# sidfeels/cosmos-predict2.5

Measured on AMD Instinct MI355X. Metric: frames/sec, Predict2.5-2B Image2World 720p×121f, 35 UniPC steps, CP=1/8, higher is better.
Workload: dtype bf16

## Files before the change

cosmos-predict2.5_amd/csrc/attn_wide.hip:

```cpp
#include "attn_common.h"

namespace cp25attn {
namespace {

constexpr int kAheadWq = 2;
constexpr int kRingWq = kAheadWq + 1;
static_assert(kWqThreads == 4 * 64, "one wave per SIMD");

constexpr int wq_stage(int nq) { return 17 * nq; }
constexpr int wq_frag(int nq, int m) { return m < nq ? -1 : (m - nq) / nq; }
constexpr int wq_qb(int nq, int m) { return m < nq ? m : (m - nq) % nq; }
constexpr bool wq_read_gap(int nq, int m) { return m >= nq && (m - nq) % nq == 0; }
constexpr int wq_sm_op(int nq, int m) {
  if (wq_read_gap(nq, m)) return -1;
  int idx = 0;
  for (int x = 0; x < m; ++x) idx += !wq_read_gap(nq, x);
  return idx < 12 * nq ? idx : -1;
}
constexpr int wq_sm_count(int nq) {
  int n = 0;
  for (int m = 0; m < wq_stage(nq); ++m) n += wq_sm_op(nq, m) >= 0;
  return n;
}
static_assert(wq_sm_count(5) == 60 && wq_sm_count(6) == 72, "every softmax instruction has a gap");
#ifdef CP25_WQ_PARENT_LOOP
#define CP25_WQ_ITER_TILES 1
#undef CP25_WQ_NO_PAD_FETCH
#undef CP25_WQ_GAP_RSRC
#endif
#ifndef CP25_WQ_ITER_TILES
#define CP25_WQ_ITER_TILES 2
#endif
constexpr int wq_iter_tiles(int) { return CP25_WQ_ITER_TILES; }
#ifdef CP25_WQ_NO_PAD_FETCH
constexpr bool kWqPadFetch = false;
#else
constexpr bool kWqPadFetch = true;
#endif
#ifdef CP25_WQ_GAP_RSRC
constexpr bool kWqHeadRsrc = false;
#else
constexpr bool kWqHeadRsrc = true;
#endif
constexpr int kWqImg = kKBuf16;
static_assert(kKBuf16 == kVBuf16, "K and V images of one size");
constexpr int wq_dma_n(int it) { return it == 1 ? 10 : 18; }
constexpr int wq_dma_at(int nq, int it, int M) {
  const int st = M / wq_stage(nq), m = M % wq_stage(nq);
  if (st >= 2 * it || !wq_read_gap(nq, m)) return -1;
  const int F = 16 * st + wq_frag(nq, m);
  return F < wq_dma_n(it) ? F : -1;
}
constexpr int wq_m0_at(int nq, int it, int M) { return wq_dma_at(nq, it, M + 1); }
constexpr int kWqNoFetch = 0x7ffffff0;

__device__ __forceinline__ u32x4 tile_rsrc(const char* base, int64_t sl, int rows) {
  const uint64_t p = (uint64_t)base;
  const unsigned n = rows > 0 ? (unsigned)((rows - 1) * sl * 2 + 2 * kD) : 0u;
  return u32x4{(unsigned)p, (unsigned)(p >> 32) & 0xffffu, n, 0x00020000u};
}

#define WQ_MFMA "v_mfma_f32_16x16x32_bf16 "

template <int kNQ, int kMode, int kTail = 0>
__global__ void __launch_bounds__(kWqThreads, 1) attn_fwd_wq(AttnArgs a) {
  static_assert(kMode == 0 || kMode == 1, "kMode: 0 fixed shift, 1 zero shift");
  static_assert(kNQ >= 4 && kNQ <= 6, "query blocks per wave");
  constexpr int kIT = wq_iter_tiles(kNQ);
  static_assert(kIT == 1 || kIT == 2, "tiles per iteration");
  constexpr int kBuf = kIT * kWqImg;
  constexpr int VB0 = 2 * kBuf;
  static_assert(4 * kBuf <= 163840, "the CU's LDS");
  __shared__ __attribute__((aligned(16))) char smem[4 * kBuf];
  constexpr bool kInit = kMode != 1;
  constexpr int kPar = kIT == 1 ? 1 : 0;
  constexpr int kND = wq_dma_n(kIT);
  constexpr int kR = kRingWq;
  constexpr int kRowsW = 16 * kNQ;
  constexpr int kRowsG = 4 * kRowsW;
  constexpr int kNS = wq_stage(kNQ);
  constexpr int kQA = (256 - 36 * kNQ - 4) / 16 < kNQ ? (256 - 36 * kNQ - 4) / 16 : kNQ;

  const int tile = xcd_remap(blockIdx.x, gridDim.x);
  const int qblk = tile % a.nqb;
  const int bhs = tile / a.nqb;
  const int split = bhs % a.nsplit, bh = bhs / a.nsplit;
  const int b = bh / a.H, h = bh % a.H;
  const int key0 = split * a.tps * kKBlk;
  const int Lk = min(a.Lk - key0, a.tps * kKBlk);
  const int ntk = (Lk + kKBlk - 1) / kKBlk;
  const int tid = threadIdx.x;
  const int lane = tid & 63;
  const int wave = __builtin_amdgcn_readfirstlane(tid >> 6);
  const int c16 = lane & 15;
  const int g = lane >> 4;
  const int row_w = qblk * kRowsG + wave * kRowsW;

  const unsigned short* qp = a.q + b * a.q_sb + h * a.q_sh;
  const char* const kbase = (const char*)(a.k + b * a.k_sb + h * a.k_sh + (int64_t)key0 * a.k_sl);
  const char* const vbase = (const char*)(a.v + b * a.v_sb + h * a.v_sh + (int64_t)key0 * a.v_sl);

  const int wave5 = kIT == 1 ? wave : (wave & 1);
  const int img5 = kIT == 1 ? 0 : (wave >> 1);
  int dk[5], dv[5];
#pragma unroll
  for (int j = 0; j < 5; ++j) {
    const int bb = 1024 * ((j < 4 ? wave : wave5) + 4 * j) + 16 * lane;
    const int row = bb / kKStride16, cb = bb - row * kKStride16;
    dk[j] = cb < 2 * kD ? row * (int)(a.k_sl * 2) + cb : (kWqPadFetch ? 0 : kWqNoFetch);
    dv[j] = cb < 2 * kD ? row * (int)(a.v_sl * 2) + cb : (kWqPadFetch ? 0 : kWqNoFetch);
  }
  const unsigned lds_wave = (unsigned)(uintptr_t)(lds_char_ptr)smem + 1024u * (unsigned)wave;
  const unsigned lds_wave5 =
      (unsigned)(uintptr_t)(lds_char_ptr)smem + 1024u * (unsigned)wave5 + (unsigned)kWqImg * (unsigned)img5;
  auto k_rsrc = [&](int t) __attribute__((always_inline)) {
    return tile_rsrc(kbase + (int64_t)t * kKBlk * a.k_sl * 2, a.k_sl, min(Lk - t * kKBlk, kKBlk));
  };
  auto v_rsrc = [&](int t) __attribute__((always_inline)) {
    return tile_rsrc(vbase + (int64_t)t * kKBlk * a.v_sl * 2, a.v_sl, min(Lk - t * kKBlk, kKBlk));
  };
  auto set_m0 = [&](unsigned dst, auto OFFC) __attribute__((always_inline)) {
    asm volatile("s_add_u32 m0, %0, %1" ::"s"(dst), "i"(decltype(OFFC)::value) : "memory", "scc");
  };
  auto dma_load = [&](const u32x4& rs, int off) __attribute__((always_inline)) {
    asm volatile("buffer_load_dwordx4 %0, %1, 0 offen lds" ::"v"(off), "s"(rs) : "memory");
  };
  auto dma_piece = [&](const u32x4& rs, int off, unsigned dst, auto OFFC) __attribute__((always_inline)) {
    set_m0(dst, OFFC);
    asm volatile("s_nop 4" ::: "memory");
    dma_load(rs, off);
  };
  auto dma_img = [&](const u32x4& rs, const int* offs, unsigned at) __attribute__((always_inline)) {
    static_for<4>([&](auto JC) __attribute__((always_inline)) {
      dma_piece(rs, offs[decltype(JC)::value], lds_wave + at, std::integral_constant<int, 4096 * decltype(JC)::value>{});
    });
  };
  auto dma_buf = [&](auto rsrc, const int* offs, int t0, unsigned at) __attribute__((always_inline)) {
    if constexpr (kIT == 1) {
      const u32x4 rs = rsrc(t0);
      dma_img(rs, offs, at);
      if (wave < 2) dma_piece(rs, offs[4], lds_wave + at, std::integral_constant<int, 16384>{});
    } else {
      const u32x4 rs0 = rsrc(t0), rs1 = rsrc(t0 + 1);
      dma_img(rs0, offs, at);
      dma_img(rs1, offs, at + (unsigned)kWqImg);
      if (wave < 2) dma_piece(rs0, offs[4], lds_wave5 + at, std::integral_constant<int, 16384>{});
      else dma_piece(rs1, offs[4], lds_wave5 + at, std::integral_constant<int, 16384>{});
    }
  };

  constexpr unsigned kK0At = (unsigned)(((kPar + 1) & 1) * kBuf + (kIT - 1) * kWqImg);
  {
    const u32x4 rs = k_rsrc(0);
    dma_img(rs, dk, kK0At);
    if (wave < 2) dma_piece(rs, dk[4], lds_wave + kK0At, std::integral_constant<int, 16384>{});
  }
  dma_buf(k_rsrc, dk, 1, (unsigned)((kPar & 1) * kBuf));
  dma_buf(v_rsrc, dv, 0, (unsigned)VB0);

  bf16x8 qa[kNQ][4];
#pragma unroll
  for (int qb = 0; qb < kNQ; ++qb) {
    const int r = row_w + 16 * qb + c16;
    const unsigned short* src = qp + (int64_t)min(r, a.Lq - 1) * a.q_sl + 8 * g;
#pragma unroll
    for (int s = 0; s < 4; ++s) qa[qb][s] = *reinterpret_cast<const bf16x8*>(src + 32 * s);
  }
  if (a.qn_w != nullptr) {
    bf16x8 wv[4];
#pragma unroll
    for (int s = 0; s < 4; ++s) wv[s] = *reinterpret_cast<const bf16x8*>(a.qn_w + 32 * s + 8 * g);
    const bool rope = a.qn_cos != nullptr;
    const f32x2 scale2 = {a.qn_scale, a.qn_scale};
#pragma unroll
    for (int qb = 0; qb < kNQ; ++qb) {
      const int r = row_w + 16 * qb + c16;
      f32x4 rc[2][2], rsn[2][2];
      if (rope) {
        const int64_t t0 = (a.qn_row0 + min(r, a.Lq - 1)) * 64 + 8 * g;
#pragma unroll
        for (int s1 = 0; s1 < 2; ++s1)
#pragma unroll
          for (int hf = 0; hf < 2; ++hf) {
            rc[s1][hf] = *reinterpret_cast<const f32x4*>(a.qn_cos + t0 + 32 * s1 + 4 * hf);
            rsn[s1][hf] = *reinterpret_cast<const f32x4*>(a.qn_sin + t0 + 32 * s1 + 4 * hf);
          }
      }
      f32x2 x[4][4];
#pragma unroll
      for (int s = 0; s < 4; ++s)
#pragma unroll
        for (int q = 0; q < 4; ++q)
          x[s][q] = f32x2{static_cast<float>(qa[qb][s][2 * q]), static_cast<float>(qa[qb][s][2 * q + 1])};
      f32x2 c01[8], c23[8];
#pragma unroll
      for (int e = 0; e < 8; ++e) {
        c01[e] = f32x2{x[0][e >> 1][e & 1], x[1][e >> 1][e & 1]};
        c23[e] = f32x2{x[2][e >> 1][e & 1], x[3][e >> 1][e & 1]};
      }
      const f32x2 p01 = hn2_sumsq8(c01), p23 = hn2_sumsq8(c23);
      const f32x2 aa = p01 + p23;
      float ss = aa.x + aa.y;
      ss += __shfl_xor(ss, 32);
      ss += __shfl_xor(ss, 16);
      const float rstd = hn_rstd(ss, a.qn_eps);
      const f32x2 rstd2 = {rstd, rstd};
#pragma unroll
      for (int s = 0; s < 4; ++s)
#pragma unroll
        for (int q = 0; q < 4; ++q)
          x[s][q] = hn2_norm(x[s][q], rstd2,
                             f32x2{static_cast<float>(wv[s][2 * q]), static_cast<float>(wv[s][2 * q + 1])});
      f32x2 y[4][4];
#pragma unroll
      for (int s = 0; s < 4; ++s)
#pragma unroll
        for (int q = 0; q < 4; ++q) y[s][q] = x[s][q];
      if (rope) {
#pragma unroll
        for (int s = 0; s < 4; ++s)
#pragma unroll
          for (int q = 0; q < 4; ++q) {
            const f32x4 cc = rc[s & 1][q >> 1], sn = rsn[s & 1][q >> 1];
            const int o = 2 * (q & 1);
            y[s][q] = hn2_rope(x[s][q], x[s ^ 2][q], s < 2 ? -1.f : 1.f, f32x2{cc[o], cc[o + 1]},
                               f32x2{sn[o], sn[o + 1]});
          }
      }
#pragma unroll
      for (int s = 0; s < 4; ++s)
#pragma unroll
        for (int q = 0; q < 4; ++q) {
          const bf16x2v hh = __builtin_convertvector(y[s][q] * scale2, bf16x2v);
          qa[qb][s][2 * q] = hh.x;
          qa[qb][s][2 * q + 1] = hh.y;
        }
    }
  }

  float m_run[kNQ];
#pragma unroll
  for (int qb = 0; qb < kNQ; ++qb) m_run[qb] = 0.f;
  if constexpr (kMode == 0) {
#pragma unroll
    for (int qb = 0; qb < kNQ; ++qb) {
      float qq = 0.f;
#pragma unroll
      for (int s = 0; s < 4; ++s)
#pragma unroll
        for (int e = 0; e < 8; ++e) {
          const float x = static_cast<float>(qa[qb][s][e]);
          qq = fmaf(x, x, qq);
        }
      const float b_row = sqrtf(group4_sum(qq)) * a.kbound;
      m_run[qb] = floorf(fminf(b_row + kPDrop, 126.f - b_row));
    }
  }
  f32x4 minit[kNQ];
#pragma unroll
  for (int qb = 0; qb < kNQ; ++qb) {
    minit[qb] = f32x4{-m_run[qb], -m_run[qb], -m_run[qb], -m_run[qb]};
    asm volatile("" : "+v"(minit[qb]));
  }

  f32x4 oacc[8][kNQ], lacc[kNQ];
#pragma unroll
  for (int db = 0; db < 8; ++db)
#pragma unroll
    for (int qb = 0; qb < kNQ; ++qb) {
      oacc[db][qb] = f32x4{0.f, 0.f, 0.f, 0.f};
      asm volatile("s_nop 2" : "+a"(oacc[db][qb]));
    }
#pragma unroll
  for (int qb = 0; qb < kNQ; ++qb) {
    lacc[qb] = f32x4{0.f, 0.f, 0.f, 0.f};
    asm volatile("s_nop 2" : "+a"(lacc[qb]));
  }
  static_for<kNQ>([&](auto QC) __attribute__((always_inline)) {
    constexpr int qb = decltype(QC)::value;
    (void)qa;
#pragma unroll
    for (int s = 0; s < 4; ++s) {
      if constexpr (qb < kQA) asm volatile("s_nop 2" : "+a"(qa[qb][s]));
      else asm volatile("s_nop 2" : "+v"(qa[qb][s]));
    }
  });
  typedef short s16x8v __attribute__((ext_vector_type(8)));
  bf16x8 ones8 = __builtin_bit_cast(bf16x8, s16x8v{0x3f80, 0x3f80, 0x3f80, 0x3f80, 0x3f80, 0x3f80, 0x3f80, 0x3f80});
  asm volatile("s_nop 2" : "+a"(ones8));
  const unsigned k_rd_lds = (unsigned)(uintptr_t)(lds_char_ptr)(smem + c16 * kKStride16 + 16 * g);
  const unsigned v_rd_lds =
      (unsigned)(uintptr_t)(lds_char_ptr)(smem + VB0 + (4 * g + (c16 >> 2)) * kVStride16 + 8 * (c16 & 3));

  f32x4 S[2][2][kNQ];
  bf16x8 P[2][kNQ];
  bf16x8 ring[kR];
  float ex[2];
  unsigned pk[4];
  unsigned k_cur = 0, v_cur = 0;

  auto issue = [&](auto FC, auto SLOTC) __attribute__((always_inline)) {
    constexpr int F = decltype(FC)::value, slot = decltype(SLOTC)::value;
    constexpr int st = F / 16, f = F % 16;
    constexpr int img = (st >> 1) * kWqImg, hs = st & 1;
    static_assert(img + kWqImg <= 65536, "ds_read offset field");
    (void)ring;
    (void)k_cur;
    (void)v_cur;
    if constexpr (f >= 8) {
      constexpr int j = f - 8;
      constexpr int off = img + (2 * hs + (j & 1)) * 16 * kKStride16 + 64 * (j >> 1);
      asm volatile("ds_read_b128 %0, %1 offset:%2" : "=v"(ring[slot]) : "v"(k_cur), "i"(off));
    } else {
      constexpr int off = img + 32 * hs * kVStride16 + 32 * f;
      s16x4 lo, hi;
      asm volatile("ds_read_b64_tr_b16 %0, %1 offset:%2" : "=v"(lo) : "v"(v_cur), "i"(off));
      asm volatile("ds_read_b64_tr_b16 %0, %1 offset:%2" : "=v"(hi) : "v"(v_cur), "i"(off + 16 * kVStride16));
      typedef short s16x8 __attribute__((ext_vector_type(8)));
      const s16x8 r = {lo[0], lo[1], lo[2], lo[3], hi[0], hi[1], hi[2], hi[3]};
      ring[slot] = __builtin_bit_cast(bf16x8, r);
    }
  };

  auto mask_keys = [&](auto SPC, int k0) __attribute__((always_inline)) {
    constexpr int SP = decltype(SPC)::value;
    if (__builtin_expect(k0 + 32 > Lk, 0)) {
      asm volatile("s_nop 15\n\ts_nop 15" ::: "memory");
#pragma unroll
      for (int kbl = 0; kbl < 2; ++kbl)
#pragma unroll
        for (int i = 0; i < 4; ++i)
          if (k0 + 16 * kbl + 4 * g + i >= Lk) {
#pragma unroll
            for (int qb = 0; qb < kNQ; ++qb) S[SP][kbl][qb][i] = -INFINITY;
          }
    }
  };

  u32x4 rk[kIT], rv[kIT], rk5 = {0u, 0u, 0u, 0u}, rv5 = {0u, 0u, 0u, 0u};
  const int64_t kstep = (int64_t)kKBlk * a.k_sl * 2, vstep = (int64_t)kKBlk * a.v_sl * 2;
  const char* kp = kbase + (kIT + 1) * kstep;
  const char* vp = vbase + kIT * vstep;
  int rows_k = Lk - (kIT + 1) * kKBlk, rows_v = Lk - kIT * kKBlk;
  auto dma_next = [&](auto CC) __attribute__((always_inline)) {
    constexpr int c = decltype(CC)::value;
    if constexpr (c == 0) {
#pragma unroll
      for (int i = 0; i < kIT; ++i) rk[i] = tile_rsrc(kp + i * kstep, a.k_sl, min(rows_k - i * kKBlk, kKBlk));
      kp += kIT * kstep;
      rows_k -= kIT * kKBlk;
    } else if constexpr (c == 1) {
#pragma unroll
      for (int i = 0; i < kIT; ++i) rv[i] = tile_rsrc(vp + i * vstep, a.v_sl, min(rows_v - i * kKBlk, kKBlk));
      vp += kIT * vstep;
      rows_v -= kIT * kKBlk;
    } else if constexpr (kIT == 2) {
#pragma unroll
      for (int e = 0; e < 4; ++e) {
        rk5[e] = img5 ? rk[kIT - 1][e] : rk[0][e];
        rv5[e] = img5 ? rv[kIT - 1][e] : rv[0][e];
      }
    }
  };
  if constexpr (!kWqHeadRsrc) static_for<3>(dma_next);
  constexpr int kNextAt = (2 * kIT - 1) * wq_stage(kNQ) + wq_stage(kNQ) - 3;
  static_assert(!wq_read_gap(kNQ, wq_stage(kNQ) - 3) && !wq_read_gap(kNQ, wq_stage(kNQ) - 2) &&
                    !wq_read_gap(kNQ, wq_stage(kNQ) - 1) && wq_sm_op(kNQ, wq_stage(kNQ) - 3) < 0,
                "a stage's last three gaps carry no read and no softmax instruction");

  auto body = [&](auto FULLC, int t) __attribute__((always_inline)) {
    constexpr bool FULL = decltype(FULLC)::value;
    constexpr int NST = FULL ? 2 * kIT : 2;
    constexpr int NF = FULL ? 16 * NST : 16;
    constexpr auto frag_of = [](int n) constexpr { return FULL ? n : (n < 8 ? 8 + n : 16 + n); };
    constexpr auto seq_of = [](int F) constexpr { return FULL ? F : (F < 16 ? F - 8 : F - 16); };
    constexpr auto nreads = [](int F) constexpr { return F % 16 < 8 ? 2 : 1; };
    const int key_sm = FULL ? 64 * kIT * t + 32 : -32;
    unsigned dst_k = 0, dst_v = 0, dst_k5 = 0, dst_v5 = 0;
    if constexpr (FULL) {
      k_cur = k_rd_lds + (((t + kPar) & 1) ? (unsigned)kBuf : 0u);
      v_cur = v_rd_lds + ((t & 1) ? (unsigned)kBuf : 0u);
      mask_keys(std::integral_constant<int, 1>{}, key_sm);
      if constexpr (kWqHeadRsrc) {
#pragma unroll
        for (int i = 0; i < kIT; ++i) {
          rk[i] = k_rsrc(kIT * (t + 1) + 1 + i);
          rv[i] = v_rsrc(kIT * (t + 1) + i);
        }
        if constexpr (kIT == 2) dma_next(std::integral_constant<int, 2>{});
      }
      const unsigned at_k = ((t + 1 + kPar) & 1) ? (unsigned)kBuf : 0u;
      const unsigned at_v = (unsigned)VB0 + (((t + 1) & 1) ? (unsigned)kBuf : 0u);
      dst_k = lds_wave + at_k;
      dst_v = lds_wave + at_v;
      if constexpr (kIT == 2) {
        dst_k5 = lds_wave5 + at_k;
        dst_v5 = lds_wave5 + at_v;
      }
    } else {
      k_cur = k_rd_lds + kK0At;
      v_cur = v_rd_lds;
    }
    auto dma_m0 = [&](auto DC) __attribute__((always_inline)) {
      constexpr int d = decltype(DC)::value, i = d % (kND / 2);
      constexpr bool isk = d < kND / 2;
      (void)dst_k;
      (void)dst_v;
      (void)dst_k5;
      (void)dst_v5;
      if constexpr (kIT == 1) {
        if (i < 4 || wave < 2) set_m0(isk ? dst_k : dst_v, std::integral_constant<int, 4096 * i>{});
      } else if constexpr (i < 8) {
        set_m0(isk ? dst_k : dst_v, std::integral_constant<int, (i / 4) * kWqImg + 4096 * (i % 4)>{});
      } else {
        set_m0(isk ? dst_k5 : dst_v5, std::integral_constant<int, 16384>{});
      }
    };
    auto dma_ld = [&](auto DC) __attribute__((always_inline)) {
      constexpr int d = decltype(DC)::value, i = d % (kND / 2);
      constexpr bool isk = d < kND / 2;
      (void)rk;
      (void)rv;
      (void)rk5;
      (void)rv5;
      if constexpr (kIT == 1) {
        if (i < 4 || wave < 2) dma_load(isk ? rk[0] : rv[0], isk ? dk[i] : dv[i]);
      } else if constexpr (i < 8) {
        dma_load(isk ? rk[i / 4] : rv[i / 4], isk ? dk[i % 4] : dv[i % 4]);
      } else {
        dma_load(isk ? rk5 : rv5, isk ? dk[4] : dv[4]);
      }
    };
    static_for<kAheadWq>([&](auto IC) __attribute__((always_inline)) {
      constexpr int n = decltype(IC)::value;
      issue(std::integral_constant<int, frag_of(n)>{}, std::integral_constant<int, n % kR>{});
    });
    __builtin_amdgcn_sched_barrier(0);
    static_for<NST * kNS>([&](auto MC) __attribute__((always_inline)) {
      constexpr int M = decltype(MC)::value;
      constexpr int st = M / kNS, m = M % kNS, hs = st & 1;
      constexpr int f = wq_frag(kNQ, m), qb = wq_qb(kNQ, m);
      constexpr int F = 16 * st + (f < 0 ? 0 : f);
      constexpr bool has_mfma = f >= 8 || FULL;
      constexpr bool has_sm = st >= 1 || FULL;
      (void)S;
      (void)ex;
      (void)pk;
      (void)oacc;
      (void)lacc;
      (void)ones8;
      (void)P;
      (void)minit;
      (void)qa;
      (void)ring;
      if constexpr (m == 0 && st >= 1) {
        if constexpr (!FULL) asm volatile("s_nop 15" ::: "memory");
        mask_keys(std::integral_constant<int, 1 - hs>{}, key_sm + 32 * st);
        __builtin_amdgcn_sched_barrier(0);
      }
      if constexpr (has_mfma) {
        if constexpr (f >= 0 && qb == 0) {
          constexpr int n = seq_of(F);
          constexpr int pending = [=]() constexpr {
            int p = 0;
            for (int i = 1; i < kAheadWq; ++i)
              if (n + i < NF) p += nreads(frag_of(n + i));
            return p;
          }();
          asm volatile("s_waitcnt lgkmcnt(%0)" ::"i"(pending), "v"(ring[n % kR]) : "memory");
        }
        if constexpr (f < 0) {
          asm volatile(WQ_MFMA "%0, %1, %2, %0" : "+a"(lacc[qb]) : "a"(ones8), "v"(P[hs][qb]));
        } else if constexpr (f < 8) {
          asm volatile(WQ_MFMA "%0, %1, %2, %0" : "+a"(oacc[f][qb]) : "v"(ring[seq_of(F) % kR]), "v"(P[hs][qb]));
        } else {
          constexpr int kbl = (f - 8) & 1, s = (f - 8) >> 1;
          constexpr int ri = seq_of(F) % kR;
          if constexpr (qb < kQA) {
            if constexpr (s == 0 && kInit)
              asm volatile(WQ_MFMA "%0, %1, %2, %3"
                           : "=&v"(S[hs][kbl][qb]) : "v"(ring[ri]), "a"(qa[qb][s]), "v"(minit[qb]));
            else if constexpr (s == 0)
              asm volatile(WQ_MFMA "%0, %1, %2, 0" : "=&v"(S[hs][kbl][qb]) : "v"(ring[ri]), "a"(qa[qb][s]));
            else
              asm volatile(WQ_MFMA "%0, %1, %2, %0" : "+v"(S[hs][kbl][qb]) : "v"(ring[ri]), "a"(qa[qb][s]));
          } else {
            if constexpr (s == 0 && kInit)
              asm volatile(WQ_MFMA "%0, %1, %2, %3"
                           : "=&v"(S[hs][kbl][qb]) : "v"(ring[ri]), "v"(qa[qb][s]), "v"(minit[qb]));
            else if constexpr (s == 0)
              asm volatile(WQ_MFMA "%0, %1, %2, 0" : "=&v"(S[hs][kbl][qb]) : "v"(ring[ri]), "v"(qa[qb][s]));
            else
              asm volatile(WQ_MFMA "%0, %1, %2, %0" : "+v"(S[hs][kbl][qb]) : "v"(ring[ri]), "v"(qa[qb][s]));
          }
        }
      }
      __builtin_amdgcn_sched_barrier(0);
      if constexpr (has_mfma && f >= 0 && qb == 0) {
        constexpr int n = seq_of(F) + kAheadWq;
        if constexpr (n < NF) issue(std::integral_constant<int, frag_of(n)>{}, std::integral_constant<int, n % kR>{});
      }
      if constexpr (FULL) {
        constexpr int dm = wq_m0_at(kNQ, kIT, M), dl = wq_dma_at(kNQ, kIT, M);
        if constexpr (dm >= 0) dma_m0(std::integral_constant<int, dm>{});
        if constexpr (dl >= 0) dma_ld(std::integral_constant<int, dl>{});
        if constexpr (!kWqHeadRsrc && M >= kNextAt && M < kNextAt + 3)
          dma_next(std::integral_constant<int, M - kNextAt>{});
      }
      if constexpr (has_sm) {
        if constexpr (!has_mfma) asm volatile("s_nop 1" ::: "memory");
        constexpr int op = wq_sm_op(kNQ, m);
        if constexpr (op >= 0) {
          constexpr int q = op / 12, r = op % 12, pair = r / 3, w = r % 3;
          if constexpr (w < 2) {
            constexpr int j = 2 * pair + w;
            asm volatile("v_exp_f32 %0, %1" : "=v"(ex[w]) : "v"(S[1 - hs][j >> 2][q][j & 3]));
          } else {
            pk[pair] = __builtin_bit_cast(unsigned, __builtin_convertvector(f32x2{ex[0], ex[1]}, bf16x2v));
            asm volatile("" ::"v"(pk[pair]));
            if constexpr (pair == 3) P[1 - hs][q] = __builtin_bit_cast(bf16x8, u32x4{pk[0], pk[1], pk[2], pk[3]});
          }
        }
      }
      __builtin_amdgcn_sched_barrier(0);
    });
    if constexpr (FULL) {
      static_for<kNQ>([&](auto QC) __attribute__((always_inline)) {
        constexpr int qb = decltype(QC)::value;
        (void)P;
        asm volatile("" ::"v"(P[0][qb]), "v"(P[1][qb]));
      });
    }
    asm volatile("s_waitcnt vmcnt(0)" ::: "memory");
    __builtin_amdgcn_s_barrier();
    __builtin_amdgcn_sched_barrier(0);
  };

  asm volatile("s_waitcnt vmcnt(0) lgkmcnt(0)" ::: "memory");
  __builtin_amdgcn_s_barrier();
  body(std::false_type{}, -1);
  const int nit = (ntk + kIT - 1) / kIT;
  for (int t = 0; t < nit; ++t) body(std::true_type{}, t);

  asm volatile("s_nop 15\n\ts_nop 15" ::: "memory");
#pragma unroll
  for (int db = 0; db < 8; ++db)
#pragma unroll
    for (int qb = 0; qb < kNQ; ++qb) asm volatile("s_nop 0" : "+a"(oacc[db][qb]));
#pragma unroll
  for (int qb = 0; qb < kNQ; ++qb) asm volatile("s_nop 0" : "+a"(lacc[qb]));
#pragma unroll
  for (int qb = 0; qb < kNQ; ++qb) {
    const int q_row = row_w + 16 * qb + c16;
    const float l_tot = lacc[qb][0];
    float inv = 1.f / l_tot;
    if (l_tot > 3.0e38f) inv = __uint_as_float(0x7fc00000u);
    if (q_row >= a.Lq) continue;
    if (a.nsplit > 1) {
      const int64_t row = ((int64_t)(split * a.B + b) * a.H + h) * a.Lq + q_row;
      float* op = a.o_part + row * kD + 4 * g;
#pragma unroll
      for (int db = 0; db < 8; ++db) {
        f32x4 w;
#pragma unroll
        for (int e = 0; e < 4; ++e) w[e] = oacc[db][qb][e] * inv;
        *reinterpret_cast<f32x4*>(op + 16 * db) = w;
      }
      if (g == 0) a.lse_part[row] = m_run[qb] + __log2f(l_tot);
    } else {
      unsigned short* op = a.o + b * a.o_sb + h * a.o_sh + (int64_t)q_row * a.o_sl + 4 * g;
#pragma unroll
      for (int db = 0; db < 8; ++db) {
        u16x4 w;
#pragma unroll
        for (int e = 0; e < 4; ++e) w[e] = f2bf(oacc[db][qb][e] * inv);
        *reinterpret_cast<u16x4*>(op + 16 * db) = w;
      }
    }
  }
}

#undef WQ_MFMA

}

AttnKernel wq_kernel(int rows, int mode, bool tail) {
  if (mode != 0) return nullptr;
  if (rows == 320) return tail ? attn_fwd_wq<5, 0, 1> : attn_fwd_wq<5, 0>;
  if (rows == 384) return tail ? attn_fwd_wq<6, 0, 1> : attn_fwd_wq<6, 0>;
  return nullptr;
}

}
```

Measured before the change: 0.8312.

## Use a dense swizzled LDS image for K/V tiles instead of a padded-stride image

Adds a new LDS image layout for K/V tiles. Each tile is 16 pieces of 1 KB at a 1056-byte stride, with rows interleaved so that every DMA piece covers whole rows and the ds_read immediates stay lane-uniform. The old layout used a padded row stride, which needed a fifth partial DMA piece per image and pad fetches. The new one makes the default path 4 pieces per image with no extra pad loads and no rk5/rv5 descriptor shuffling. The padded layout is kept behind a macro. The change risks different LDS bank conflict behaviour for the MFMA fragment reads and transposed V reads.

After: 0.8466, median of 6. +1.8%, better.

```diff
diff --git a/cosmos-predict2.5_amd/csrc/attn_wide.hip b/cosmos-predict2.5_amd/csrc/attn_wide.hip
--- a/cosmos-predict2.5_amd/csrc/attn_wide.hip
+++ b/cosmos-predict2.5_amd/csrc/attn_wide.hip
@@ -1,4 +1,5 @@
 #include "attn_common.h"
+#include "attn_wq_image.h"
 
 namespace cp25attn {
 namespace {
@@ -25,26 +26,33 @@
 static_assert(wq_sm_count(5) == 60 && wq_sm_count(6) == 72, "every softmax instruction has a gap");
 #ifdef CP25_WQ_PARENT_LOOP
 #define CP25_WQ_ITER_TILES 1
-#undef CP25_WQ_NO_PAD_FETCH
-#undef CP25_WQ_GAP_RSRC
+#ifndef CP25_WQ_PAD_IMAGE
+#define CP25_WQ_PAD_IMAGE
+#endif
+#ifndef CP25_WQ_HEAD_RSRC
+#define CP25_WQ_HEAD_RSRC
+#endif
 #endif
 #ifndef CP25_WQ_ITER_TILES
 #define CP25_WQ_ITER_TILES 2
 #endif
 constexpr int wq_iter_tiles(int) { return CP25_WQ_ITER_TILES; }
-#ifdef CP25_WQ_NO_PAD_FETCH
-constexpr bool kWqPadFetch = false;
+#ifdef CP25_WQ_PAD_IMAGE
+constexpr bool kWqPad = true;
 #else
-constexpr bool kWqPadFetch = true;
+constexpr bool kWqPad = false;
 #endif
-#ifdef CP25_WQ_GAP_RSRC
+#ifdef CP25_WQ_HEAD_RSRC
+constexpr bool kWqHeadRsrc = true;
+#else
 constexpr bool kWqHeadRsrc = false;
-#else
-constexpr bool kWqHeadRsrc = true;
 #endif
-constexpr int kWqImg = kKBuf16;
 static_assert(kKBuf16 == kVBuf16, "K and V images of one size");
-constexpr int wq_dma_n(int it) { return it == 1 ? 10 : 18; }
+constexpr int kWqImg = kWqPad ? kKBuf16 : wqimg::kImage;
+constexpr int kWqPieceAt = kWqPad ? 1024 : wqimg::kPieceStride;
+constexpr int kWqPieceStep = 4 * kWqPieceAt;
+constexpr int kWqOffs = kWqPad ? 5 : 4;
+constexpr int wq_dma_n(int it) { return !kWqPad ? 8 * it : it == 1 ? 10 : 18; }
 constexpr int wq_dma_at(int nq, int it, int M) {
   const int st = M / wq_stage(nq), m = M % wq_stage(nq);
   if (st >= 2 * it || !wq_read_gap(nq, m)) return -1;
@@ -52,7 +60,6 @@
   return F < wq_dma_n(it) ? F : -1;
 }
 constexpr int wq_m0_at(int nq, int it, int M) { return wq_dma_at(nq, it, M + 1); }
-constexpr int kWqNoFetch = 0x7ffffff0;
 
 __device__ __forceinline__ u32x4 tile_rsrc(const char* base, int64_t sl, int rows) {
   const uint64_t p = (uint64_t)base;
@@ -72,6 +79,12 @@
   constexpr int VB0 = 2 * kBuf;
   static_assert(4 * kBuf <= 163840, "the CU's LDS");
   __shared__ __attribute__((aligned(16))) char smem[4 * kBuf];
+  static_assert(kWqPad || 3 * kBuf + (kIT - 1) * kWqImg + wqimg::piece_dst(wqimg::wave_piece(3, 3)) +
+                                  wqimg::kPieceBytes <= 4 * kBuf,
+                "every DMA piece lands inside smem");
+  static_assert(kWqPad || (wqimg::piece_dst(wqimg::wave_piece(1, 0)) == kWqPieceAt &&
+                           wqimg::piece_dst(wqimg::wave_piece(0, 1)) == kWqPieceStep),
+                "a wave's piece destinations: base + step j");
   constexpr bool kInit = kMode != 1;
   constexpr int kPar = kIT == 1 ? 1 : 0;
   constexpr int kND = wq_dma_n(kIT);
@@ -102,16 +115,23 @@
 
   const int wave5 = kIT == 1 ? wave : (wave & 1);
   const int img5 = kIT == 1 ? 0 : (wave >> 1);
-  int dk[5], dv[5];
-#pragma unroll
-  for (int j = 0; j < 5; ++j) {
-    const int bb = 1024 * ((j < 4 ? wave : wave5) + 4 * j) + 16 * lane;
-    const int row = bb / kKStride16, cb = bb - row * kKStride16;
-    dk[j] = cb < 2 * kD ? row * (int)(a.k_sl * 2) + cb : (kWqPadFetch ? 0 : kWqNoFetch);
-    dv[j] = cb < 2 * kD ? row * (int)(a.v_sl * 2) + cb : (kWqPadFetch ? 0 : kWqNoFetch);
-  }
-  const unsigned lds_wave = (unsigned)(uintptr_t)(lds_char_ptr)smem + 1024u * (unsigned)wave;
-  const unsigned lds_wave5 =
+  int dk[kWqOffs], dv[kWqOffs];
+#pragma unroll
+  for (int j = 0; j < kWqOffs; ++j) {
+    if constexpr (kWqPad) {
+      const int bb = 1024 * ((j < 4 ? wave : wave5) + 4 * j) + 16 * lane;
+      const int row = bb / kKStride16, cb = bb - row * kKStride16;
+      dk[j] = cb < 2 * kD ? row * (int)(a.k_sl * 2) + cb : 0;
+      dv[j] = cb < 2 * kD ? row * (int)(a.v_sl * 2) + cb : 0;
+    } else {
+      const int P = wqimg::wave_piece(wave, j);
+      const int row = wqimg::piece_row(P, lane), cb = wqimg::piece_col(lane);
+      dk[j] = row * (int)(a.k_sl * 2) + cb;
+      dv[j] = row * (int)(a.v_sl * 2) + cb;
+    }
+  }
+  const unsigned lds_wave = (unsigned)(uintptr_t)(lds_char_ptr)smem + (unsigned)kWqPieceAt * (unsigned)wave;
+  [[maybe_unused]] const unsigned lds_wave5 =
       (unsigned)(uintptr_t)(lds_char_ptr)smem + 1024u * (unsigned)wave5 + (unsigned)kWqImg * (unsigned)img5;
   auto k_rsrc = [&](int t) __attribute__((always_inline)) {
     return tile_rsrc(kbase + (int64_t)t * kKBlk * a.k_sl * 2, a.k_sl, min(Lk - t * kKBlk, kKBlk));
@@ -132,11 +152,15 @@
   };
   auto dma_img = [&](const u32x4& rs, const int* offs, unsigned at) __attribute__((always_inline)) {
     static_for<4>([&](auto JC) __attribute__((always_inline)) {
-      dma_piece(rs, offs[decltype(JC)::value], lds_wave + at, std::integral_constant<int, 4096 * decltype(JC)::value>{});
+      dma_piece(rs, offs[decltype(JC)::value], lds_wave + at,
+                std::integral_constant<int, kWqPieceStep * decltype(JC)::value>{});
     });
   };
   auto dma_buf = [&](auto rsrc, const int* offs, int t0, unsigned at) __attribute__((always_inline)) {
-    if constexpr (kIT == 1) {
+    if constexpr (!kWqPad) {
+#pragma unroll
+      for (int i = 0; i < kIT; ++i) dma_img(rsrc(t0 + i), offs, at + (unsigned)(i * kWqImg));
+    } else if constexpr (kIT == 1) {
       const u32x4 rs = rsrc(t0);
       dma_img(rs, offs, at);
       if (wave < 2) dma_piece(rs, offs[4], lds_wave + at, std::integral_constant<int, 16384>{});
@@ -153,7 +177,8 @@
   {
     const u32x4 rs = k_rsrc(0);
     dma_img(rs, dk, kK0At);
-    if (wave < 2) dma_piece(rs, dk[4], lds_wave + kK0At, std::integral_constant<int, 16384>{});
+    if constexpr (kWqPad)
+      if (wave < 2) dma_piece(rs, dk[kWqOffs - 1], lds_wave + kK0At, std::integral_constant<int, 16384>{});
   }
   dma_buf(k_rsrc, dk, 1, (unsigned)((kPar & 1) * kBuf));
   dma_buf(v_rsrc, dv, 0, (unsigned)VB0);
@@ -288,9 +313,12 @@
   typedef short s16x8v __attribute__((ext_vector_type(8)));
   bf16x8 ones8 = __builtin_bit_cast(bf16x8, s16x8v{0x3f80, 0x3f80, 0x3f80, 0x3f80, 0x3f80, 0x3f80, 0x3f80, 0x3f80});
   asm volatile("s_nop 2" : "+a"(ones8));
-  const unsigned k_rd_lds = (unsigned)(uintptr_t)(lds_char_ptr)(smem + c16 * kKStride16 + 16 * g);
+  const unsigned k_rd_lds =
+      (unsigned)(uintptr_t)(lds_char_ptr)smem +
+      (unsigned)(kWqPad ? c16 * kKStride16 + 16 * g : wqimg::k_lane_base(lane));
   const unsigned v_rd_lds =
-      (unsigned)(uintptr_t)(lds_char_ptr)(smem + VB0 + (4 * g + (c16 >> 2)) * kVStride16 + 8 * (c16 & 3));
+      (unsigned)(uintptr_t)(lds_char_ptr)smem + (unsigned)VB0 +
+      (unsigned)(kWqPad ? (4 * g + (c16 >> 2)) * kVStride16 + 8 * (c16 & 3) : wqimg::v_lane_base(lane));
 
   f32x4 S[2][2][kNQ];
   bf16x8 P[2][kNQ];
@@ -309,13 +337,17 @@
     (void)v_cur;
     if constexpr (f >= 8) {
       constexpr int j = f - 8;
-      constexpr int off = img + (2 * hs + (j & 1)) * 16 * kKStride16 + 64 * (j >> 1);
+      constexpr int kb = 2 * hs + (j & 1), s = j >> 1;
+      constexpr int off = img + (kWqPad ? kb * 16 * kKStride16 + 64 * s : wqimg::k_imm(kb, s));
+      static_assert(off < 65536, "ds_read offset field");
       asm volatile("ds_read_b128 %0, %1 offset:%2" : "=v"(ring[slot]) : "v"(k_cur), "i"(off));
     } else {
-      constexpr int off = img + 32 * hs * kVStride16 + 32 * f;
+      constexpr int off = img + (kWqPad ? 32 * hs * kVStride16 + 32 * f : wqimg::v_imm(hs, 0, f));
+      constexpr int off_hi = img + (kWqPad ? (32 * hs + 16) * kVStride16 + 32 * f : wqimg::v_imm(hs, 1, f));
+      static_assert(off_hi < 65536, "ds_read offset field");
       s16x4 lo, hi;
       asm volatile("ds_read_b64_tr_b16 %0, %1 offset:%2" : "=v"(lo) : "v"(v_cur), "i"(off));
-      asm volatile("ds_read_b64_tr_b16 %0, %1 offset:%2" : "=v"(hi) : "v"(v_cur), "i"(off + 16 * kVStride16));
+      asm volatile("ds_read_b64_tr_b16 %0, %1 offset:%2" : "=v"(hi) : "v"(v_cur), "i"(off_hi));
       typedef short s16x8 __attribute__((ext_vector_type(8)));
       const s16x8 r = {lo[0], lo[1], lo[2], lo[3], hi[0], hi[1], hi[2], hi[3]};
       ring[slot] = __builtin_bit_cast(bf16x8, r);
@@ -337,7 +369,8 @@
     }
   };
 
-  u32x4 rk[kIT], rv[kIT], rk5 = {0u, 0u, 0u, 0u}, rv5 = {0u, 0u, 0u, 0u};
+  u32x4 rk[kIT], rv[kIT];
+  [[maybe_unused]] u32x4 rk5 = {0u, 0u, 0u, 0u}, rv5 = {0u, 0u, 0u, 0u};
   const int64_t kstep = (int64_t)kKBlk * a.k_sl * 2, vstep = (int64_t)kKBlk * a.v_sl * 2;
   const char* kp = kbase + (kIT + 1) * kstep;
   const char* vp = vbase + kIT * vstep;
@@ -354,7 +387,7 @@
       for (int i = 0; i < kIT; ++i) rv[i] = tile_rsrc(vp + i * vstep, a.v_sl, min(rows_v - i * kKBlk, kKBlk));
       vp += kIT * vstep;
       rows_v -= kIT * kKBlk;
-    } else if constexpr (kIT == 2) {
+    } else if constexpr (kWqPad && kIT == 2) {
 #pragma unroll
       for (int e = 0; e < 4; ++e) {
         rk5[e] = img5 ? rk[kIT - 1][e] : rk[0][e];
@@ -387,13 +420,13 @@
           rk[i] = k_rsrc(kIT * (t + 1) + 1 + i);
           rv[i] = v_rsrc(kIT * (t + 1) + i);
         }
-        if constexpr (kIT == 2) dma_next(std::integral_constant<int, 2>{});
+        if constexpr (kWqPad && kIT == 2) dma_next(std::integral_constant<int, 2>{});
       }
       const unsigned at_k = ((t + 1 + kPar) & 1) ? (unsigned)kBuf : 0u;
       const unsigned at_v = (unsigned)VB0 + (((t + 1) & 1) ? (unsigned)kBuf : 0u);
       dst_k = lds_wave + at_k;
       dst_v = lds_wave + at_v;
-      if constexpr (kIT == 2) {
+      if constexpr (kWqPad && kIT == 2) {
         dst_k5 = lds_wave5 + at_k;
         dst_v5 = lds_wave5 + at_v;
       }
@@ -408,10 +441,10 @@
       (void)dst_v;
       (void)dst_k5;
       (void)dst_v5;
-      if constexpr (kIT == 1) {
+      if constexpr (kWqPad && kIT == 1) {
         if (i < 4 || wave < 2) set_m0(isk ? dst_k : dst_v, std::integral_constant<int, 4096 * i>{});
-      } else if constexpr (i < 8) {
-        set_m0(isk ? dst_k : dst_v, std::integral_constant<int, (i / 4) * kWqImg + 4096 * (i % 4)>{});
+      } else if constexpr (i < 4 * kIT) {
+        set_m0(isk ? dst_k : dst_v, std::integral_constant<int, (i / 4) * kWqImg + kWqPieceStep * (i % 4)>{});
       } else {
         set_m0(isk ? dst_k5 : dst_v5, std::integral_constant<int, 16384>{});
       }
@@ -423,12 +456,12 @@
       (void)rv;
       (void)rk5;
       (void)rv5;
-      if constexpr (kIT == 1) {
+      if constexpr (kWqPad && kIT == 1) {
         if (i < 4 || wave < 2) dma_load(isk ? rk[0] : rv[0], isk ? dk[i] : dv[i]);
-      } else if constexpr (i < 8) {
+      } else if constexpr (i < 4 * kIT) {
         dma_load(isk ? rk[i / 4] : rv[i / 4], isk ? dk[i % 4] : dv[i % 4]);
       } else {
-        dma_load(isk ? rk5 : rv5, isk ? dk[4] : dv[4]);
+        dma_load(isk ? rk5 : rv5, isk ? dk[kWqOffs - 1] : dv[kWqOffs - 1]);
       }
     };
     static_for<kAheadWq>([&](auto IC) __attribute__((always_inline)) {
diff --git a/cosmos-predict2.5_amd/csrc/attn_wq_image.h b/cosmos-predict2.5_amd/csrc/attn_wq_image.h
--- /dev/null
+++ b/cosmos-predict2.5_amd/csrc/attn_wq_image.h
@@ -0,0 +1,62 @@
+#pragma once
+
+namespace cp25attn {
+namespace wqimg {
+
+constexpr int kRows = 64;
+constexpr int kRowBytes = 256;
+constexpr int kPieceBytes = 1024;
+constexpr int kPieceStride = 1056;
+constexpr int kPieces = 16;
+constexpr int kGroupStride = 8 * kPieceStride;
+constexpr int kImage = 2 * kGroupStride;
+constexpr int kWaves = 4;
+constexpr int kWaveStep = kWaves * kPieceStride;
+
+constexpr int off(int row, int col) {
+  return kGroupStride * (row >> 5) + kPieceStride * (row & 7) + kRowBytes * ((row & 31) >> 3) + col;
+}
+
+constexpr int piece_dst(int P) { return kPieceStride * P; }
+constexpr int piece_row(int P, int lane) { return 32 * (P >> 3) + (P & 7) + 8 * (lane >> 4); }
+constexpr int piece_col(int lane) { return 16 * (lane & 15); }
+constexpr int wave_piece(int wave, int j) { return wave + kWaves * j; }
+constexpr int piece_of(int row) { return 8 * (row >> 5) + (row & 7); }
+constexpr int lane_of(int row, int chunk) { return 16 * ((row & 31) >> 3) + chunk; }
+
+constexpr int k_lane_base(int lane) { return off(lane & 15, 16 * (lane >> 4)); }
+constexpr int k_imm(int kb, int s) { return kGroupStride * (kb >> 1) + 2 * kRowBytes * (kb & 1) + 64 * s; }
+constexpr int v_lane_row(int lane) { return 4 * (lane >> 4) + ((lane & 15) >> 2); }
+constexpr int v_lane_base(int lane) { return off(v_lane_row(lane), 8 * (lane & 3)); }
+constexpr int v_imm(int ks, int hf, int f) { return kGroupStride * ks + 2 * kRowBytes * hf + 32 * f; }
+
+constexpr bool reads_consistent() {
+  for (int lane = 0; lane < 64; ++lane) {
+    for (int kb = 0; kb < 4; ++kb)
+      for (int s = 0; s < 4; ++s)
+        if (k_lane_base(lane) + k_imm(kb, s) != off(16 * kb + (lane & 15), 64 * s + 16 * (lane >> 4))) return false;
+    for (int ks = 0; ks < 2; ++ks)
+      for (int hf = 0; hf < 2; ++hf)
+        for (int f = 0; f < 8; ++f)
+          if (v_lane_base(lane) + v_imm(ks, hf, f) !=
+              off(32 * ks + 16 * hf + v_lane_row(lane), 32 * f + 8 * (lane & 3)))
+            return false;
+  }
+  return true;
+}
+constexpr bool pieces_consistent() {
+  for (int P = 0; P < kPieces; ++P) {
+    if (piece_dst(P) + kPieceBytes > kImage) return false;
+    for (int lane = 0; lane < 64; ++lane) {
+      const int row = piece_row(P, lane), col = piece_col(lane);
+      if (row < 0 || row >= kRows || piece_of(row) != P || lane_of(row, col / 16) != lane) return false;
+      if (off(row, col) != piece_dst(P) + 16 * lane) return false;
+    }
+  }
+  return true;
+}
+static_assert(reads_consistent(), "the fragment reads' immediates are lane-uniform");
+static_assert(pieces_consistent(), "16 pieces of 64 chunks tile the image");
+
+}
+}
```
